# gaetanfacchinetti/DensityFlows.jl

Measured on AMD Instinct MI355X. Metric: forward+logdetJ Msamples/s, d=5 8-layer RealNVP, 1/2/4/8 MI355X, higher is better.
Workload: dtype f32

## Files before the change

densityflows.jl_amd/csrc/df_plan.cpp:

```cpp
#include "df_plan.h"

#include <algorithm>
#include <cmath>
#include <cstring>
#include <cstdlib>
#include <set>
#include <sstream>

namespace df {
namespace {

struct Fail {
    int code;
    std::string msg;
};

[[noreturn]] void fail(int code, const std::string& m) { throw Fail{code, m}; }

int round_up(int v, int m) { return (v + m - 1) / m * m; }

int pow2_tiles(int t) {
    int p = 1;
    while (p < t) p *= 2;
    return p;
// ... 47 lines not shown
private:
    Plan& P;
    int cap_;
    int cur_ = -1;
    int used_ = 0;
};

void check_net(const df_dense_desc* net, int nd, int in_dim, int out_dim, const char* which) {
    if (nd < 1) fail(DF_ERR_INVALID, std::string(which) + ": a conditioner needs at least one Dense");
    if (!net) fail(DF_ERR_INVALID, std::string(which) + ": null Dense array");
    int prev = in_dim;
    for (int k = 0; k < nd; ++k) {
        const df_dense_desc& D = net[k];
        if (D.in_dim != prev) {
            std::ostringstream os;
            os << which << ": Dense " << k + 1 << " expects " << D.in_dim << " inputs but receives " << prev;
            fail(DF_ERR_SHAPE, os.str());
        }
        if (D.out_dim < 1 || !D.W) fail(DF_ERR_INVALID, std::string(which) + ": empty Dense");
        if (D.act < DF_ACT_IDENTITY || D.act > DF_ACT_SWISH)
            fail(DF_ERR_INVALID, std::string(which) + ": unknown activation");
        if (k + 1 < nd && D.out_dim > kMaxHidden) fail(DF_ERR_UNSUPPORTED, "hidden width > 256");
        prev = D.out_dim;
    }
    if (prev != out_dim) {
        std::ostringstream os;
        os << which << ": output dimension " << prev << " does not match the " << out_dim
           << " transformed dimensions";
        fail(DF_ERR_SHAPE, os.str());
    }
}

void build_split(const df_chain_desc* desc, Plan& P, const std::vector<char>& fold) {
    P.split = 0;
    if (!P.fast || (P.ht != 2 && P.ht != 4)) return;
    const int ht = P.ht, H = 16 * ht;
    auto net_bytes = [&](int n_out) {
        return kSplitFirstBytes(ht) + kSplitHiddenBytes(ht) + 4 * H + round_up((n_out * H + 4) * 4, 16);
    };
    int total = 0, biggest = 0;
    for (const ULayer& U : P.ulayers) {
        if (U.kind == DF_LAYER_NORM) continue;
        const int b = net_bytes(U.t.n_out) + (U.kind == DF_LAYER_RNVP ? net_bytes(U.s.n_out) : 0);
        total += b;
        biggest = std::max(biggest, std::max(net_bytes(U.t.n_out), U.kind == DF_LAYER_RNVP ? net_bytes(U.s.n_out) : 0));
    }
    const int cap = total <= kSingleStageCap ? kSingleStageCap : std::max(kStageCap, round_up(biggest, kStageAlign));
    std::vector<uint8_t>& blob = P.sblob;
    int cur = -1, used = 0;
    auto close = [&]() {
        if (cur < 0) return;
        used = round_up(used, kStageAlign);
        blob.resize((size_t)P.sstages[cur].src_off + used, 0);
        P.sstages[cur].bytes = used;
        P.sstage_max = std::max(P.sstage_max, used);
    };
    auto alloc = [&](int bytes) {
        if (cur < 0 || used + bytes > cap) {
            close();
            cur = (int)P.sstages.size();
            DevStage s{};
            s.src_off = (int64_t)blob.size();
            P.sstages.push_back(s);
            used = 0;
        }
        const int off = used;
        used += bytes;
        blob.resize((size_t)P.sstages[cur].src_off + used, 0);
        return std::make_pair(cur, off);
    };
    P.sulayers = P.ulayers;
    for (int li = 0; li < desc->n_layers; ++li) {
        const df_layer_desc& L = desc->layers[li];
        if (L.kind == DF_LAYER_NORM) continue;
        const DevLayer& DL = P.layers[li];
        auto pack = [&](const df_dense_desc* net, int d0, UNet* u) {
            const DevDense &D0 = P.denses[d0], &D1 = P.denses[d0 + 1], &DO = P.denses[d0 + 2];
            auto [st, off] = alloc(net_bytes(u->n_out));
            u->stage = st;
            u->off_w0 = off;
            u->off_h = off + kSplitFirstBytes(ht);
            u->off_out = u->off_h + kSplitHiddenBytes(ht) + 4 * H;
            u->off_b0 = -1;
            u->hstride = 0;
            const int64_t base = P.sstages[st].src_off;
            auto put16 = [&](int64_t at, int32_t src, int plane, float v) {
                const uint16_t h = bf16_split_plane(v, plane);
                std::memcpy(&blob[base + at], &h, 2);
                if (src >= 0) {
                    P.spack_dst.push_back((int32_t)(base + at));
                    P.spack_src.push_back(src * 4 + plane);
                }
            };
            auto put32 = [&](int64_t at, int32_t src, float v) {
                std::memcpy(&blob[base + at], &v, 4);
                if (src >= 0) {
                    P.spack_dst.push_back((int32_t)(base + at));
                    P.spack_src.push_back(src * 4 + 3);
                }
            };
            const df_dense_desc& W0 = net[0];
            static const int kPlaneOfSlot[6] = {0, 0, 1, 0, 1, 2};
            for (int m = 0; m < ht; ++m)
                for (int lane = 0; lane < 64; ++lane) {
                    const int g = lane >> 4, row = 16 * m + (lane & 15);
                    float v = 0.f;
                    int32_t src = -1;
                    if (row < W0.out_dim) {
                        if (fold[li] && g == 3) {
                            v = W0.b[row];
                            src = D0.b_off + row;
                        } else if (g < W0.in_dim) {
                            v = W0.W[(size_t)row + (size_t)W0.out_dim * g];
                            src = D0.w_off + row + W0.out_dim * g;
                        }
                    }
                    for (int e = 0; e < 6; ++e)
                        put16(u->off_w0 + ((int64_t)m * 64 + lane) * 16 + 2 * e, src, kPlaneOfSlot[e], v);
                }
            const df_dense_desc& W1 = net[1];
            for (int c = 0; c < ht / 2; ++c)
                for (int m = 0; m < ht; ++m)
                    for (int p = 0; p < 3; ++p)
                        for (int lane = 0; lane < 64; ++lane)
                            for (int e = 0; e < 8; ++e) {
                                const int g = lane >> 4, row = 16 * m + (lane & 15);
                                const int k = 32 * c + 16 * (e >> 2) + 4 * g + (e & 3);
                                const bool ok = row < W1.out_dim && k < W1.in_dim;
                                put16(u->off_h + ((((int64_t)c * ht + m) * 3 + p) * 64 + lane) * 16 + 2 * e,
                                      ok ? D1.w_off + row + W1.out_dim * k : -1, p,
                                      ok ? W1.W[(size_t)row + (size_t)W1.out_dim * k] : 0.f);
                            }
            const int64_t hb = u->off_h + kSplitHiddenBytes(ht);
            for (int row = 0; row < H; ++row) {
                const bool ok = W1.b && row < W1.out_dim;
                put32(hb + 4 * row, ok ? D1.b_off + row : -1, ok ? W1.b[row] : 0.f);
            }
            const df_dense_desc& W2 = net[2];
            for (int o = 0; o < W2.out_dim; ++o)
                for (int k = 0; k < H; ++k) {
                    const bool ok = k < W2.in_dim;
                    put32(u->off_out + 4 * ((int64_t)o * H + k), ok ? DO.w_off + o + W2.out_dim * k : -1,
                          ok ? W2.W[(size_t)o + (size_t)W2.out_dim * k] : 0.f);
                }
            for (int o = 0; o < 4; ++o) {
                const bool ok = W2.b && o < W2.out_dim;
                put32(u->off_out + 4 * ((int64_t)W2.out_dim * H + o), ok ? DO.b_off + o : -1, ok ? W2.b[o] : 0.f);
            }
            P.split_flops_per_sample += 2.0 * (W0.in_dim * W0.out_dim + W1.in_dim * W1.out_dim);
        };
        ULayer& U = P.sulayers[li];
        if (L.kind == DF_LAYER_RNVP) pack(L.s_net, DL.s_dense0, &U.s);
        pack(L.t_net, DL.t_dense0, &U.t);
    }
    close();
    auto sched = [&](bool fwd) {
        std::vector<int32_t> out;
        auto push = [&](int s) {
            if (out.empty() || out.back() != s) out.push_back(s);
        };
        for (int it = 0; it < P.n_layers; ++it) {
            const ULayer& U = P.sulayers[fwd ? it : P.n_layers - 1 - it];
            if (U.kind == DF_LAYER_NORM) continue;
            if (fwd) {
                if (U.kind == DF_LAYER_RNVP) push(U.s.stage);
                push(U.t.stage);
            } else {
                push(U.t.stage);
                if (U.kind == DF_LAYER_RNVP) push(U.s.stage);
            }
        }
        return out;
    };
    P.ssched_fwd = sched(true);
    P.ssched_bwd = sched(false);
    int target = kLdsPerBlockTarget;
    if (const char* e = std::getenv("DF_SPLIT_LDS_KB")) target = std::max(32, std::atoi(e)) * 1024;
    const int nbuf = P.sstages.size() > 1 ? 2 : 1;
    const int fixed = nbuf * P.sstage_max + table_lds_bytes(P);
    const int per_tile = kWavesPerBlock * 16 * P.stride * 4;
    int t = 0;
    while (t < kMaxTilesPerWave && fixed + (t + 1) * per_tile <= target) ++t;
    t -= t % P.tile_group;
    if (t < P.tile_group) {
        P.sulayers.clear();
        P.sstages.clear();
        P.sblob.clear();
        P.spack_dst.clear();
        P.spack_src.clear();
        P.split_flops_per_sample = 0.0;
        return;
    }
    P.stiles = t;
    P.sblob.resize(round_up((int)P.sblob.size(), 16) + 16, 0);
    P.split = 1;
}

void build_wide(const df_chain_desc* desc, Plan& P) {
    if (const char* f = std::getenv("DF_NO_WIDE"))
        if (f[0] == '1') return;
    if (P.uniform || P.ht != 16) return;
    for (int li = 0; li < desc->n_layers; ++li) {
        const df_layer_desc& L = desc->layers[li];
        if (L.kind == DF_LAYER_NORM) continue;
        auto ok = [&](const df_dense_desc* net, int nd) {
            return nd == 3 && net[0].in_dim <= kMaxState && net[0].out_dim == 256 && net[1].out_dim == 256 &&
                   net[2].out_dim <= 32 && net[0].act == DF_ACT_RELU && net[1].act == DF_ACT_RELU &&
                   net[2].act == DF_ACT_IDENTITY;
        };
        if (L.kind == DF_LAYER_RNVP && !ok(L.s_net, L.n_dense_s)) return;
        if (!ok(L.t_net, L.n_dense_t)) return;
    }
    int li_dense = 0;
    std::vector<WLayer> wl;
    for (int li = 0; li < desc->n_layers; ++li) {
        const df_layer_desc& L = desc->layers[li];
        const DevLayer& DL = P.layers[li];
        WLayer W{};
        W.kind = DL.kind;
        W.elem_start = DL.elem_start;
        W.elem_end = DL.elem_end;
        W.n_af = DL.n_af;
        W.feat_tab = DL.feat_tab;
        W.af_tab = DL.af_tab;
        W.norm_off = DL.norm_off;
        W.alpha = DL.alpha;
        W.beta = DL.beta;
        W.ldj_const = DL.ldj_const;
        if (L.kind != DF_LAYER_NORM) {
            auto pack = [&](const df_dense_desc* net, int d0, WNet& N) {
                const int ks = (net[0].in_dim + 3) / 4;
                const int nkq0 = (ks + 3) / 4;
                N.stage0 = (int)P.wstages.size();
                N.nst0 = (nkq0 + 1) / 2;
                N.ks = ks;
                N.n_out = net[2].out_dim;
                N.mto = (N.n_out + 15) / 16;
                N.act0 = net[0].act;
                N.act1 = net[1].act;
                N.act_out = net[2].act;
                auto new_stage = [&](int bytes) -> float* {
                    DevStage st{};
                    st.src_off = (int64_t)P.wblob.size();
                    st.bytes = bytes;
                    P.wstages.push_back(st);
                    P.wblob.resize(P.wblob.size() + bytes, 0);
                    return reinterpret_cast<float*>(P.wblob.data() + st.src_off);
                };
                auto put = [&](float* base, int64_t q, int dense, int row, int k) {
                    const df_dense_desc& D = net[dense];
                    if (row >= D.out_dim || k >= D.in_dim) return;
                    base[q] = D.W[(size_t)row + (size_t)D.out_dim * k];
                    const int64_t f0 = (reinterpret_cast<uint8_t*>(base) - P.wblob.data()) / 4;
                    P.wpack_dst.push_back((int32_t)(f0 + q));
                    P.wpack_src.push_back(P.denses[d0 + dense].w_off + row + D.out_dim * k);
                };
                for (int st = 0; st < N.nst0; ++st) {
                    float* b = new_stage(kWideStageBytes);
                    for (int kk = 0; kk < 2; ++kk)
                        for (int m = 0; m < 16; ++m)
                            for (int lane = 0; lane < 64; ++lane)
                                for (int r = 0; r < 4; ++r) {
                                    const int s = 4 * (2 * st + kk) + r;
                                    if (s >= ks) continue;
                                    put(b, ((int64_t)(kk * 16 + m) * 64 + lane) * 4 + r, 0, 16 * m + (lane & 15),
                                        4 * s + (lane >> 4));
                                }
                }
                for (int st = 0; st < 8; ++st) {
                    float* b = new_stage(kWideStageBytes);
                    for (int kk = 0; kk < 2; ++kk)
                        for (int m = 0; m < 16; ++m)
                            for (int lane = 0; lane < 64; ++lane)
                                for (int r = 0; r < 4; ++r)
                                    put(b, ((int64_t)(kk * 16 + m) * 64 + lane) * 4 + r, 1, 16 * m + (lane & 15),
                                        16 * (2 * st + kk) + 4 * (lane >> 4) + r);
                }
                {
                    float* b = new_stage(16 * N.mto * 1024);
                    for (int kq = 0; kq < 16; ++kq)
                        for (int m = 0; m < N.mto; ++m)
                            for (int lane = 0; lane < 64; ++lane)
                                for (int r = 0; r < 4; ++r)
                                    put(b, ((int64_t)(kq * N.mto + m) * 64 + lane) * 4 + r, 2, 16 * m + (lane & 15),
                                        16 * kq + 4 * (lane >> 4) + r);
                }
                auto bias = [&](int dense, int rows) -> int32_t {
                    const df_dense_desc& D = net[dense];
                    const int32_t off = (int32_t)P.wbias.size();
                    P.wbias.resize(P.wbias.size() + rows, 0.f);
                    if (!D.b) return off;
                    for (int r = 0; r < D.out_dim; ++r) {
                        P.wbias[off + r] = D.b[r];
                        P.wbias_dst.push_back(off + r);
                        P.wbias_src.push_back(P.denses[d0 + dense].b_off + r);
                    }
                    return off;
                };
                N.b0 = bias(0, 256);
                N.b1 = bias(1, 256);
                N.bo = bias(2, 16 * N.mto);
            };
            if (L.kind == DF_LAYER_RNVP) pack(L.s_net, DL.s_dense0, W.s);
            pack(L.t_net, DL.t_dense0, W.t);
        }
        wl.push_back(W);
// ... 653 lines not shown
```

densityflows.jl_amd/csrc/df_plan.h:

```cpp
#pragma once

#include <cstdint>
#include <string>
#include <vector>

#include "densityflows_hip.h"

namespace df {

constexpr int kWave = 64;
#ifndef DF_BLOCK_WAVES
#define DF_BLOCK_WAVES 8
#endif
#ifndef DF_LDS_TARGET_KB
#define DF_LDS_TARGET_KB 80
#endif
constexpr int kBlockThreads = 64 * DF_BLOCK_WAVES;
constexpr int kWavesPerBlock = kBlockThreads / kWave;
constexpr int kMaxState = 64;
constexpr int kMaxHidden = 256;
constexpr int kMaxAf = 32;
constexpr int kMaxLayers = 4096;
constexpr int kStageCap = 24 * 1024;
constexpr int kSingleStageCap = 64 * 1024;
constexpr int kBigStageCap = 64 * 1024;
constexpr int kStageAlign = 1024;
constexpr int kMaxTableInts = 4096;
constexpr int kMaxTilesPerWave = 8;
#ifndef DF_UNI_TT
#define DF_UNI_TT 1
#endif
constexpr int kUniformTileGroup = DF_UNI_TT;
#ifndef DF_FAST_TT
#define DF_FAST_TT 2
#endif
constexpr int kFastTileGroup = DF_FAST_TT;
constexpr int kLdsPerBlockTarget = DF_LDS_TARGET_KB * 1024;

enum : int32_t { IN_STATE = 0, IN_HIDDEN = 1 };

struct DevChunk {
    int32_t stage, lds_off, kq_begin, kq_end;
};

struct DevDense {
    int32_t in_kind;
    int32_t ks;
    int32_t kt_in;
    int32_t mt;
    int32_t out_valu;
    int32_t n_out;
    int32_t act;
    int32_t has_bias;
    int32_t bias_stage, bias_lds;
    int32_t chunk0, n_chunks;
    int32_t w3_stage, w3_lds;
    int32_t compact;
    int32_t in_dim;
    int32_t w_off, b_off;
};

struct DevLayer {
    int32_t kind;
    int32_t elem_start;
    int32_t elem_end;
    int32_t n_af;
    int32_t feat_tab;
    int32_t af_tab;
    int32_t s_dense0, s_ndense;
    int32_t t_dense0, t_ndense;
    int32_t norm_off;
    int32_t out_valu;
    float alpha, beta, ldj_const, pad;
};

struct UNet {
    int32_t stage;
    int32_t ks;
    int32_t nh;
    int32_t n_out;
    int32_t off_w0, off_b0;
    int32_t off_h, hstride;
    int32_t off_out;
    int32_t act0, acth, act_out;
    int32_t fold0;
};

struct ULayer {
    int32_t kind, elem_start, elem_end, n_af;
    int32_t feat_tab, af_tab, norm_off, pad0;
    float alpha, beta, ldj_const, pad1;
    UNet s, t;
};

constexpr int kWideStageBytes = 32 * 1024;
#ifndef DF_WIDE_NB
#define DF_WIDE_NB 2
#endif
constexpr int kWideBufs = DF_WIDE_NB;
constexpr int kWideWaves = 4;
constexpr int kWideT = 2;
#ifndef DF_WSPLIT_HALF
#define DF_WSPLIT_HALF 0
#endif
constexpr int kWideSplitHalves = DF_WSPLIT_HALF ? 2 : 1;
constexpr int kWideSplitStageBytes = 48 * 1024 / kWideSplitHalves;
constexpr int kWideSplitBufs = DF_WSPLIT_HALF ? 4 : 2;

struct WNet {
    int32_t stage0;
    int32_t nst0;
    int32_t nso;
    int32_t ks;
    int32_t n_out, mto;
    int32_t act0, act1, act_out;
    int32_t b0, b1, bo;
};

struct WLayer {
    int32_t kind, elem_start, elem_end, n_af;
    int32_t feat_tab, af_tab, norm_off, pad0;
    float alpha, beta, ldj_const, pad1;
    WNet s, t;
};

struct DevStage {
    int64_t src_off;
    int32_t bytes;
    int32_t pad;
};

#if defined(__HIPCC__)
#define DF_HD __host__ __device__
#else
#define DF_HD
#endif
DF_HD inline uint16_t bf16_rne_bits(float f) {
    const uint32_t u = __builtin_bit_cast(uint32_t, f);
    if ((u & 0x7fffffffu) > 0x7f800000u) return (uint16_t)((u >> 16) | 0x40u);
    return (uint16_t)((u + 0x7fffu + ((u >> 16) & 1u)) >> 16);
}
DF_HD inline float bf16_bits_to_f32(uint16_t h) { return __builtin_bit_cast(float, (uint32_t)h << 16); }
DF_HD inline uint16_t bf16_split_plane(float w, int plane) {
    const uint16_t h0 = bf16_rne_bits(w);
    if (plane == 0) return h0;
    const float r = w - bf16_bits_to_f32(h0);
    const uint16_t h1 = bf16_rne_bits(r);
    if (plane == 1) return h1;
    return bf16_rne_bits(r - bf16_bits_to_f32(h1));
}
constexpr int kSplitFirstBytes(int ht) { return ht * 1024; }
constexpr int kSplitHiddenBytes(int ht) { return (ht / 2) * ht * 3 * 1024; }

struct Plan {
    int d = 0, n = 0, n_layers = 0;
    int stride = 0;
    int ht = 0;
    int tiles = 0;
    int outv = 0;
    int uniform = 0;
    int relu_only = 0;
    int tile_group = 1;
    int fast = 0;
    std::vector<ULayer> ulayers;
    int samples_per_block = 0;
    int stage_max = 0;
    std::vector<int32_t> sched_fwd;
    std::vector<int32_t> sched_bwd;
    std::vector<DevLayer> layers;
    std::vector<DevDense> denses;
    std::vector<DevChunk> chunks;
    std::vector<DevStage> stages;
    std::vector<uint8_t> blob;
    std::vector<int32_t> tables;
    std::vector<float> params;
    int64_t n_params = 0;
    std::vector<float> trainables;
    std::vector<int32_t> pack_dst, pack_src;
    int wide = 0;
    std::vector<WLayer> wlayers;
    std::vector<DevStage> wstages;
    std::vector<uint8_t> wblob;
    std::vector<float> wbias;
    std::vector<int32_t> wsched_fwd, wsched_bwd;
    std::vector<int32_t> wpack_dst, wpack_src;
    std::vector<int32_t> wbias_dst, wbias_src;
    int split = 0;
    int stiles = 0;
    int sstage_max = 0;
    std::vector<ULayer> sulayers;
    std::vector<DevStage> sstages;
    std::vector<uint8_t> sblob;
    std::vector<int32_t> ssched_fwd, ssched_bwd;
    std::vector<int32_t> spack_dst, spack_src;
    int wsplit = 0;
    std::vector<WLayer> wslayers;
    std::vector<DevStage> wsstages;
    std::vector<uint8_t> wsblob;
    std::vector<int32_t> wssched_fwd, wssched_bwd;
    std::vector<int32_t> wspack_dst, wspack_src;
    std::vector<int32_t> wstables;
    double flops_per_sample = 0.0;
    double split_flops_per_sample = 0.0;
};

int build_plan(const df_chain_desc* desc, Plan* out, std::string* err, int exact = -1);

size_t plan_lds_bytes(const Plan& p);
inline bool params_in_lds(const Plan& p) { return p.uniform && p.params.size() <= (size_t)kBlockThreads; }
inline int table_lds_ints(const Plan& p) { return (int)(p.tables.size() + (params_in_lds(p) ? p.params.size() : 0)); }
inline int table_lds_bytes(const Plan& p) { return (table_lds_ints(p) * 4 + 15) / 16 * 16; }

}
```

densityflows.jl_amd/csrc/df_uniform_impl.h:

```cpp
#pragma once

#include <type_traits>

#include "df_chain_impl.h"

namespace df {
namespace uni {


using impl::lds4;
using impl::mfma4;
using impl::Stager;

__device__ __forceinline__ float relu_fast(float x) {
    return __int_as_float(__builtin_elementwise_max(__float_as_int(x), 0));
}

__device__ __forceinline__ float xgroup_sum(float p) {
    auto a = __builtin_amdgcn_permlane16_swap(__float_as_uint(p), __float_as_uint(p), false, false);
    const float q = __uint_as_float(a[0]) + __uint_as_float(a[1]);
    auto b = __builtin_amdgcn_permlane32_swap(__float_as_uint(q), __float_as_uint(q), false, false);
    return __uint_as_float(b[0]) + __uint_as_float(b[1]);
}

// ... 455 lines not shown
            const bf16x8 w2 = *reinterpret_cast<const bf16x8*>(f + 2048);
#pragma unroll
            for (int t = 0; t < TT; ++t) {
                f32x4 a = out[t][m];
                a = mfma_bf(w2, x[t][0], a);
                a = mfma_bf(w1, x[t][1], a);
                a = mfma_bf(w0, x[t][2], a);
                a = mfma_bf(w1, x[t][0], a);
                a = mfma_bf(w0, x[t][1], a);
                out[t][m] = mfma_bf(w0, x[t][0], a);
            }
            if (FENCE) asm volatile("" ::: "memory");
        }
    }
}

#ifndef DF_SPLIT_PREFETCH
#define DF_SPLIT_PREFETCH 1
#endif

__device__ __forceinline__ void sched_fence() { __builtin_amdgcn_sched_barrier(0); }

__device__ __forceinline__ void lds_wait0() { __builtin_amdgcn_s_waitcnt(0xc07f); }

struct SplitStep {
    bf16x8 w0, w1, w2;
    f32x4 b;
};

template <int HT, bool BIAS>
__device__ __forceinline__ void split_step_request(const uint8_t* wl, const uint8_t* bl, int s, SplitStep& f) {
    if (s >= (HT / 2) * HT) return;
    const uint8_t* p = wl + s * 3072;
    f.w0 = *reinterpret_cast<const bf16x8*>(p);
    f.w1 = *reinterpret_cast<const bf16x8*>(p + 1024);
    f.w2 = *reinterpret_cast<const bf16x8*>(p + 2048);
    if (BIAS && s < HT) f.b = lds4(bl + (s << 6));
}

template <int HT, int TT, bool BIAS = true>
__device__ __forceinline__ void dense_hidden_split_pf(const uint8_t* wb, int lane, const f32x4 (&in)[TT][HT],
                                                      f32x4 (&out)[TT][HT], const SplitStep& f0) {
    const int g = lane >> 4;
    const uint8_t* bl = wb + (HT / 2) * HT * 3072 + (g << 4);
    const uint8_t* wl = wb + lane * 16;
    const short4v eye = neg_eye();
    SplitStep f[2];
    f[0] = f0;
    bf16x8 x[TT][3];
#pragma unroll
    for (int s = 0; s < (HT / 2) * HT; ++s) {
        const int c = s / HT, m = s % HT;
        if (m == 0) {
#pragma unroll
            for (int t = 0; t < TT; ++t) split8_mrem(eye, in[t][2 * c], in[t][2 * c + 1], x[t][0], x[t][1], x[t][2]);
        }
        constexpr int NS = (HT / 2) * HT;
        const bool late = (m == HT - 1) && (s + 1 < NS);
        sched_fence();
        lds_wait0();
        if (!late) split_step_request<HT, BIAS>(wl, bl, s + 1, f[(s + 1) & 1]);
        sched_fence();
        const SplitStep& w = f[s & 1];
#pragma unroll
        for (int t = 0; t < TT; ++t) {
            f32x4 a = c == 0 ? (BIAS ? w.b : f32x4{0.f, 0.f, 0.f, 0.f}) : out[t][m];
            a = mfma_bf(w.w2, x[t][0], a);
            a = mfma_bf(w.w1, x[t][1], a);
            a = mfma_bf(w.w0, x[t][2], a);
            a = mfma_bf(w.w1, x[t][0], a);
            a = mfma_bf(w.w0, x[t][1], a);
            out[t][m] = mfma_bf(w.w0, x[t][0], a);
        }
        if (late) {
#pragma unroll
            for (int t = 0; t < TT; ++t) asm volatile("" : "+v"(out[t][m]));
            sched_fence();
            split_step_request<HT, BIAS>(wl, bl, s + 1, f[(s + 1) & 1]);
        }
    }
}

template <int HT, int TT>
__device__ __forceinline__ void dense_first_split_pf(const bf16x8 (&w)[HT], const float (&xin)[TT][4],
                                                     f32x4 (&acc)[TT][HT]) {
    bf16x8 b[TT];
    const __bf16 z = (__bf16)0.f;
#pragma unroll
    for (int t = 0; t < TT; t += 2) {
        bf16x2 h, m, l;
        split2(xin[t][0], t + 1 < TT ? xin[t + 1][0] : 0.f, h, m, l);
        b[t] = bf16x8{h[0], m[0], h[0], l[0], m[0], h[0], z, z};
        if (t + 1 < TT) b[t + 1] = bf16x8{h[1], m[1], h[1], l[1], m[1], h[1], z, z};
    }
#pragma unroll
    for (int m = 0; m < HT; ++m)
#pragma unroll
        for (int t = 0; t < TT; ++t) acc[t][m] = mfma_bf(w[m], b[t], f32x4{0.f, 0.f, 0.f, 0.f});
}

template <int HT, int NO>
__device__ __forceinline__ void out_row_request(const uint8_t* w3g, int oo, f32x4 (&w)[HT]) {
    if (oo >= NO) return;
#pragma unroll
    for (int kq = 0; kq < HT; ++kq) w[kq] = lds4(w3g + ((oo * 16 * HT + 16 * kq) << 2));
}

template <int HT, int TT, int NO>
__device__ __forceinline__ void out_valu_t_pf(const uint8_t* w3g, const f32x4 (&w0)[HT], float bo,
                                              const f32x4 (&h)[TT][HT], const float* state, const int (&ro)[TT],
                                              const int& aslot, float (&v)[TT], float (&y)[TT]) {
    static_assert(NO >= 1 && NO <= 4, "FAST tails: 1..4 outputs");
    float p[TT][4];
#pragma unroll
    for (int t = 0; t < TT; ++t)
#pragma unroll
        for (int oo = 0; oo < 4; ++oo) p[t][oo] = 0.f;
    f32x4 w[2][HT];
#pragma unroll
    for (int kq = 0; kq < HT; ++kq) w[0][kq] = w0[kq];
#pragma unroll
    for (int oo = 0; oo < NO; ++oo) {
        sched_fence();
        lds_wait0();
        if (oo == 0) {
#pragma unroll
            for (int t = 0; t < TT; ++t) v[t] = state[ro[t] + aslot];
        }
        out_row_request<HT, NO>(w3g, oo + 1, w[(oo + 1) & 1]);
        sched_fence();
#pragma unroll
        for (int kq = 0; kq < HT; ++kq)
#pragma unroll
            for (int r = 0; r < 4; ++r)
#pragma unroll
                for (int t = 0; t < TT; ++t) p[t][oo] = __builtin_fmaf(w[oo & 1][kq][r], h[t][kq][r], p[t][oo]);
#pragma unroll
        for (int t = 0; t < TT; ++t) asm volatile("" : "+v"(p[t][oo]));
    }
#pragma unroll
    for (int t = 0; t < TT; ++t) {
        auto a = __builtin_amdgcn_permlane16_swap(__float_as_uint(p[t][0]), __float_as_uint(p[t][1]), false, false);
        const float A = __uint_as_float(a[0]) + __uint_as_float(a[1]);
        float Bv = 0.f;
        if constexpr (NO > 2) {
            auto b = __builtin_amdgcn_permlane16_swap(__float_as_uint(p[t][2]), __float_as_uint(p[t][3]), false, false);
            Bv = __uint_as_float(b[0]) + __uint_as_float(b[1]);
        }
        auto c = __builtin_amdgcn_permlane32_swap(__float_as_uint(A), __float_as_uint(Bv), false, false);
        y[t] = (__uint_as_float(c[0]) + __uint_as_float(c[1])) + bo;
    }
}

template <int HT, int TT, bool OUTV, bool RELU, int PH, bool FAST = false, int NO = 0, bool SPLIT = false>
__device__ __forceinline__ void net_tiles(const uint8_t* buf, const UNet& N, const ULayer& L, const int32_t* tab,
                                          float* state, const int (&ro)[TT], float (&sum)[TT]) {
    const int lane = threadIdx.x & 63, g = lane >> 4;
    constexpr bool SPH = (PH == impl::PH_S_FWD || PH == impl::PH_S_BWD);
#if DF_SPLIT_PREFETCH && !defined(DF_EXP_NOTAIL) && !defined(DF_DIAG_NOSPLIT)
    if constexpr (SPLIT && FAST && HT >= 2 && OUTV && NO > 0) {
        int tx = threadIdx.x;
        asm volatile("" : "+v"(tx));
        const int lane = tx & 63, g = lane >> 4;
        const int off_out = N.off_out, af_tab = L.af_tab;
        asm volatile("" ::"s"(off_out), "s"(af_tab));
        const int slot = tab[L.feat_tab + g];
        bf16x8 w0[HT];
#pragma unroll
        for (int m = 0; m < HT; ++m) w0[m] = *reinterpret_cast<const bf16x8*>(buf + N.off_w0 + lane * 16 + m * 1024);
        sched_fence();
        lds_wait0();
        float xin[TT][4];
#pragma unroll
        for (int t = 0; t < TT; ++t) xin[t][0] = state[ro[t] + slot];
        const uint8_t* wh = buf + N.off_h;
        SplitStep f0;
        split_step_request<HT, true>(wh + lane * 16, wh + (HT / 2) * HT * 3072 + (g << 4), 0, f0);
        sched_fence();
        f32x4 A[TT][HT], B[TT][HT];
        dense_first_split_pf<HT, TT>(w0, xin, A);
        bias_act<HT, TT, true>(buf, DF_ACT_RELU, A, false);
        dense_hidden_split_pf<HT, TT>(wh, lane, A, B, f0);
        const uint8_t* w3g = buf + off_out + (g << 4);
        sched_fence();
        f32x4 wo[HT];
        out_row_request<HT, NO>(w3g, 0, wo);
        const float bo = reinterpret_cast<const float*>(buf + off_out)[NO * 16 * HT + (g < NO ? g : 0)];
        const int aslot = tab[af_tab + (g < NO ? g : 0)];
        sched_fence();
        bias_act<HT, TT, true>(buf, DF_ACT_RELU, B, false);
        float v[TT], y[TT];
        out_valu_t_pf<HT, TT, NO>(w3g, wo, bo, B, state, ro, aslot, v, y);
#pragma unroll
        for (int t = 0; t < TT; ++t) {
            if (g < NO) state[ro[t] + aslot] = couple1<PH>(v[t], y[t]);
            sum[t] = SPH ? group_row_sum<NO>(y[t]) : 0.f;
        }
        return;
    }
#endif
    if constexpr (SPLIT && FAST && HT >= 2) {
        float xin[TT][4];
        const int slot = tab[L.feat_tab + g];
#pragma unroll
        for (int t = 0; t < TT; ++t) xin[t][0] = state[ro[t] + slot];
        f32x4 A[TT][HT], B[TT][HT];
        dense_first_split<HT, TT>(buf, N, xin, A);
        bias_act<HT, TT, true>(buf, DF_ACT_RELU, A, false);
        dense_hidden_split<HT, TT>(buf + N.off_h, A, B);
        bias_act<HT, TT, true>(buf, DF_ACT_RELU, B, false);
        tail<HT, TT, OUTV, RELU, PH, NO>(buf, N, L, tab, state, ro, sum, B);
        return;
    }
    float xin[TT][4];
    const int32_t* feat = tab + L.feat_tab;
    constexpr int KS = FAST ? 1 : 0;
    const int ks = FAST ? 1 : N.ks;
#pragma unroll
    for (int r = 0; r < 4; ++r) {
        const int slot = (r < ks) ? feat[4 * r + g] : 0;
#pragma unroll
        for (int t = 0; t < TT; ++t) xin[t][r] = (r < ks) ? state[ro[t] + slot] : 0.f;
    }

    f32x4 A[TT][HT], B[TT][HT];
    dense_first<HT, TT, KS>(buf, N, xin, A);
    bias_act<HT, TT, RELU>(buf + N.off_b0, N.act0, A, FAST ? false : !N.fold0);
    if (FAST || N.nh == 1) {
        dense_hidden<HT, TT>(buf + N.off_h, A, B);
        bias_act<HT, TT, RELU>(buf + N.off_h + HT * HT * 1024, N.acth, B);
        tail<HT, TT, OUTV, RELU, PH, NO>(buf, N, L, tab, state, ro, sum, B);
        return;
    }
    bool in_a = true;
    for (int k = 0; k < N.nh; k += 2) {
        dense_hidden<HT, TT>(buf + N.off_h + k * N.hstride, A, B);
        bias_act<HT, TT, RELU>(buf + N.off_h + k * N.hstride + HT * HT * 1024, N.acth, B);
        in_a = false;
        if (k + 1 < N.nh) {
            dense_hidden<HT, TT>(buf + N.off_h + (k + 1) * N.hstride, B, A);
            bias_act<HT, TT, RELU>(buf + N.off_h + (k + 1) * N.hstride + HT * HT * 1024, N.acth, A);
            in_a = true;
        }
    }
    if (in_a) tail<HT, TT, OUTV, RELU, PH, NO>(buf, N, L, tab, state, ro, sum, A);
    else tail<HT, TT, OUTV, RELU, PH, NO>(buf, N, L, tab, state, ro, sum, B);
}

template <int HT, int TT, bool RELU, bool FWDP, int NO>
__device__ __forceinline__ void net_pair_tiles(const uint8_t* buf, const ULayer& L, const int32_t* tab, float* state,
                                               const int (&ro)[TT], float (&ssum)[TT]) {
    const int lane = threadIdx.x & 63, g = lane >> 4;
    float xin[TT][4];
    const int slot_in = tab[L.feat_tab + g];
#pragma unroll
    for (int t = 0; t < TT; ++t) xin[t][0] = state[ro[t] + slot_in];
    f32x4 As[TT][HT], At[TT][HT], Bs[TT][HT], Bt[TT][HT];
    dense_first<HT, TT, 1>(buf, L.s, xin, As);
    dense_first<HT, TT, 1>(buf, L.t, xin, At);
    bias_act<HT, TT, RELU>(buf + L.s.off_b0, L.s.act0, As, false);
    bias_act<HT, TT, RELU>(buf + L.t.off_b0, L.t.act0, At, false);
    dense_hidden<HT, TT>(buf + L.s.off_h, As, Bs);
    dense_hidden<HT, TT>(buf + L.t.off_h, At, Bt);
    bias_act<HT, TT, RELU>(buf + L.s.off_h + HT * HT * 1024, L.s.acth, Bs);
    bias_act<HT, TT, RELU>(buf + L.t.off_h + HT * HT * 1024, L.t.acth, Bt);
    float ys[TT], yt[TT];
    out_valu_t<HT, TT, NO>(buf, L.s, Bs, ys);
    out_valu_t<HT, TT, NO>(buf, L.t, Bt, yt);
    const int slot = tab[L.af_tab + (g < NO ? g : 0)];
#pragma unroll
    for (int t = 0; t < TT; ++t) {
        if (g < NO) {
            float v = state[ro[t] + slot];
            if (FWDP) {
                v = v * expf(ys[t]);
                v = v + yt[t];
            } else {
                v = v - yt[t];
                v = v * expf(-ys[t]);
            }
            state[ro[t] + slot] = v;
        }
        ssum[t] = group_row_sum<NO>(ys[t]);
    }
}

}

#ifndef DF_UNI_WAVES
#define DF_UNI_WAVES 4
#endif
#ifndef DF_FAST_WAVES
#define DF_FAST_WAVES 4
#endif

template <int HT, int MODE, bool OUTV, bool RELU, bool FAST = false, bool SPLIT = false>
__global__ void __launch_bounds__(kBlockThreads, FAST ? DF_FAST_WAVES : DF_UNI_WAVES)
uniform_kernel(ChainArgs a) {
    using namespace uni;
    constexpr bool FWD = (MODE == MODE_FWD || MODE == MODE_FWD_INPLACE);
    constexpr bool WANT_LDJ = (MODE != MODE_FWD_INPLACE);

    extern __shared__ __attribute__((aligned(16))) uint8_t smem[];
    const int stage_area = a.stage_bytes * a.n_stage_bufs;
    int32_t* tab = reinterpret_cast<int32_t*>(smem + stage_area);
    float* state = reinterpret_cast<float*>(smem + stage_area + a.tab_bytes);

    ClockStamp clk;
    clk.begin(a);
#ifdef DF_PHASE_STAMPS
    uint64_t ph[16] = {};
#define DF_PH(i) do { if (blockIdx.x == 0 && threadIdx.x == 0) ph[i] = __builtin_amdgcn_s_memtime(); } while (0)
#else
#define DF_PH(i) do {} while (0)
#endif
    DF_PH(0);
    const int tid = threadIdx.x;
    const int lane = tid & 63, wave = tid >> 6;
    const int g = lane >> 4, j = lane & 15;
    const int d = a.d, n = a.n, stride = a.stride, nd = n + d;
    const int nt = a.tiles;
    const int S = kWavesPerBlock * 16 * nt;
    const int cA = nd + 1, cE = nd + 2;
    const int64_t s0 = (int64_t)blockIdx.x * S;
    const int nvalid = (int)((a.batch - s0) < S ? (a.batch - s0) : S);

    Stager sg;
    sg.base = smem;
    sg.bytes = a.stage_bytes;
    sg.sched = FWD ? a.sched_fwd : a.sched_bwd;
    sg.n = FWD ? a.n_sched_fwd : a.n_sched_bwd;
    constexpr bool kLaneLocalDma = SPLIT && DF_SPLIT_PREFETCH;
    impl::stager_start<kLaneLocalDma>(sg, a);

    float* tabf = reinterpret_cast<float*>(tab);
    constexpr int kRowMax = 8;
    const bool fast_copy = d <= kRowMax && n <= kRowMax && a.n_par <= kBlockThreads && a.tab_ints <= 4 * kBlockThreads;
    auto row_init = [&](int smp) {
        for (int c = nd; c < stride; ++c) state[smp * stride + c] = (c == nd + 3) ? 1.f : 0.f;
    };
    auto theta_in = [&](float v, float lo, float hi) {
        const float diff = hi - lo;
        return (diff == 0.f) ? 0.f : (v - lo) / diff;
    };
    if (fast_copy) {
        const int n_tab = a.tab_ints, n_par = a.n_par;
        int tv[4];
#pragma unroll
        for (int u = 0; u < 4; ++u) {
            const int i = tid + u * kBlockThreads;
            tv[u] = i < n_tab ? a.tables[i] : 0;
        }
        const float pv = tid < n_par ? a.params[tid] : 0.f;
        const bool norm_th = a.tmin != nullptr;
        const float blo = (norm_th && lane < n) ? a.tmin[lane] : 0.f;
        const float bhi = (norm_th && lane < n) ? a.tmax[lane] : 0.f;
        const int smp = tid;
        const bool valid = smp < nvalid;
        float zr[kRowMax], tr[kRowMax];
#pragma unroll
        for (int c = 0; c < kRowMax; ++c)
            if (c < d) zr[c] = valid ? a.zin[(s0 + smp) * d + c] : 0.f;
#pragma unroll
        for (int c = 0; c < kRowMax; ++c)
            if (c < n) tr[c] = valid ? a.theta[(s0 + smp) * n + c] : 0.f;
#pragma unroll
        for (int u = 0; u < 4; ++u) {
            const int i = tid + u * kBlockThreads;
            if (i < n_tab) tab[i] = tv[u];
        }
        if (tid < n_par) tabf[n_tab + tid] = pv;
#pragma unroll
        for (int c = 0; c < kRowMax; ++c)
            if (c < n) {
                const float lo = __shfl(blo, c), hi = __shfl(bhi, c);
                if (smp < S) state[smp * stride + c] = (norm_th && valid) ? theta_in(tr[c], lo, hi) : tr[c];
            }
        if (smp < S) {
#pragma unroll
            for (int c = 0; c < kRowMax; ++c)
                if (c < d) state[smp * stride + n + c] = zr[c];
            row_init(smp);
        }
        for (int i = tid + kBlockThreads * d; i < S * d; i += kBlockThreads) {
            const int r = i / d, c = i - r * d;
            state[r * stride + n + c] = r < nvalid ? a.zin[(s0 + r) * d + c] : 0.f;
        }
        for (int i = tid + kBlockThreads * n; i < S * n; i += kBlockThreads) {
            const int r = i / n, c = i - r * n;
            float v = 0.f;
            if (r < nvalid) {
                v = a.theta[(s0 + r) * n + c];
                if (norm_th) v = theta_in(v, a.tmin[c], a.tmax[c]);
            }
            state[r * stride + c] = v;
        }
        for (int r = tid + kBlockThreads; r < S; r += kBlockThreads) row_init(r);
    } else {
        for (int i = tid; i < a.tab_ints; i += kBlockThreads) tab[i] = a.tables[i];
        for (int i = tid; i < S * d; i += kBlockThreads) {
            const int smp = i / d, c = i - smp * d;
            float v = 0.f;
            if (smp < nvalid) v = a.zin[(s0 + smp) * d + c];
            state[smp * stride + n + c] = v;
        }
        for (int i = tid; i < S * n; i += kBlockThreads) {
            const int smp = i / n, c = i - smp * n;
            float v = 0.f;
            if (smp < nvalid) {
                v = a.theta[(s0 + smp) * n + c];
                if (a.tmin) v = theta_in(v, a.tmin[c], a.tmax[c]);
            }
            state[smp * stride + c] = v;
        }
        for (int i = tid; i < S; i += kBlockThreads) row_init(i);
    }
    DF_PH(1);
    DF_PH(2);
    DF_PH(3);
    __syncthreads();
    DF_PH(4);

    const int row0 = ((wave * nt) * 16 + j) * stride;
#ifdef DF_NO_PAIR
    constexpr bool no_pair = true;
#else
    constexpr bool no_pair = false;
#endif
    const int tstep = 16 * stride;
    bool have_acc = false;

    auto ldj_update = [&](int ro, float l, bool first_in_elem, bool last_in_elem) {
        if (!WANT_LDJ || g != 0) return;
        const float e = first_in_elem ? l : state[ro + cE] + l;
        state[ro + cE] = e;
        if (last_in_elem) state[ro + cA] = have_acc ? state[ro + cA] + e : e;
    };

    for (int it = 0; it < a.n_layers; ++it) {
        const int li = FWD ? it : a.n_layers - 1 - it;
        using CULayer = const __attribute__((address_space(4))) ULayer;
#ifdef DF_PHASE_STAMPS
        const ULayer L = *(const ULayer*)(&((CULayer*)(uintptr_t)a.ulayers)[li]);
        asm volatile("s_waitcnt lgkmcnt(0)" ::: "memory");
        if (it == 1) DF_PH(13);
#else
        const ULayer& L = *(const ULayer*)(&((CULayer*)(uintptr_t)a.ulayers)[li]);
#endif
        const int kind = L.kind;
        const bool first_in_elem = FWD ? L.elem_start : L.elem_end;
        const bool last_in_elem = FWD ? L.elem_end : L.elem_start;
        int gl = g, jl = j, wavel = wave, row0l = row0;
        if constexpr (kLaneLocalDma) {
            if (kind == DF_LAYER_NORM || (!FWD && a.snap)) {
                int tx = tid;
                asm volatile("" : "+v"(tx));
                gl = (tx & 63) >> 4, jl = tx & 15, wavel = tx >> 6;
                row0l = ((wavel * nt) * 16 + jl) * stride;
            }
        }
        if (kind == DF_LAYER_NORM) {
            const float al = L.alpha, be = L.beta, delta = be - al;
            auto norm = [&](const auto* xmn) {
                const auto* xmx = xmn + d;
                for (int tt = 0; tt < nt; ++tt) {
                    const int ro = row0l + tt * tstep;
                    for (int i = gl; i < d; i += 4) {
                        const float lo = xmn[i], hi = xmx[i], xd = hi - lo;
                        float v = state[ro + n + i];
                        if (FWD) v = ((xd * v - al * hi) + be * lo) / delta;
                        else v = (be * (v - lo) + al * (hi - v)) / xd;
                        state[ro + n + i] = v;
                    }
                    ldj_update(ro, FWD ? L.ldj_const : -L.ldj_const, first_in_elem, last_in_elem);
                }
            };
            if (fast_copy) norm(tabf + a.tab_ints + L.norm_off);
            else norm(a.params + L.norm_off);
        } else {
            const bool rnvp = (kind == DF_LAYER_RNVP);
            constexpr int kTT = FAST ? kFastTileGroup : kUniformTileGroup;
            auto tiles_loop = [&](const UNet& N, auto ph_tag, auto no_tag, bool sphase, float sign) {
                constexpr int PH = decltype(ph_tag)::value;
                constexpr int NO = decltype(no_tag)::value;
                const uint8_t* buf = sg.buf();
                for (int tt = 0; tt < nt; tt += kTT) {
                    int ro[kTT];
                    float ssum[kTT];
                    int r0 = row0;
                    if constexpr (SPLIT) asm volatile("" : "+v"(r0));
#pragma unroll
                    for (int t = 0; t < kTT; ++t) ro[t] = r0 + (tt + t) * tstep;
                    net_tiles<HT, kTT, OUTV, RELU, PH, FAST, NO, SPLIT>(buf, N, L, tab, state, ro, ssum);
#pragma unroll
                    for (int t = 0; t < kTT; ++t) {
                        if (sphase) ldj_update(ro[t], sign * ssum[t], first_in_elem, last_in_elem);
                        else if (!rnvp) ldj_update(ro[t], 0.f, first_in_elem, last_in_elem);
                    }
                }
            };
            auto run_net = [&](const UNet& N, auto ph_tag, bool sphase, float sign) {
                impl::ensure_stage<kLaneLocalDma>(N.stage, sg, a);
                if constexpr (FAST && OUTV) {
                    switch (N.n_out) {
                        case 1: tiles_loop(N, ph_tag, std::integral_constant<int, 1>{}, sphase, sign); break;
                        case 2: tiles_loop(N, ph_tag, std::integral_constant<int, 2>{}, sphase, sign); break;
                        case 3: tiles_loop(N, ph_tag, std::integral_constant<int, 3>{}, sphase, sign); break;
                        default: tiles_loop(N, ph_tag, std::integral_constant<int, 4>{}, sphase, sign); break;
                    }
                } else {
                    tiles_loop(N, ph_tag, std::integral_constant<int, 0>{}, sphase, sign);
                }
            };
            using PSF = std::integral_constant<int, impl::PH_S_FWD>;
            using PTF = std::integral_constant<int, impl::PH_T_FWD>;
            using PTB = std::integral_constant<int, impl::PH_T_BWD>;
            using PSB = std::integral_constant<int, impl::PH_S_BWD>;
            bool paired = false;
            if constexpr (FAST && OUTV && !SPLIT && HT <= 2) {
                if (rnvp && L.s.stage == L.t.stage && L.s.n_out == L.t.n_out && !no_pair) {
                    impl::ensure_stage(L.s.stage, sg, a);
                    auto pair_loop = [&](auto no_tag) {
                        constexpr int NO = decltype(no_tag)::value;
                        const uint8_t* buf = sg.buf();
                        for (int tt = 0; tt < nt; tt += kTT) {
                            int ro[kTT];
                            float ssum[kTT];
#pragma unroll
                            for (int t = 0; t < kTT; ++t) ro[t] = row0 + (tt + t) * tstep;
                            net_pair_tiles<HT, kTT, RELU, FWD, NO>(buf, L, tab, state, ro, ssum);
#pragma unroll
                            for (int t = 0; t < kTT; ++t)
                                ldj_update(ro[t], FWD ? ssum[t] : -ssum[t], first_in_elem, last_in_elem);
                        }
                    };
                    switch (L.s.n_out) {
                        case 1: pair_loop(std::integral_constant<int, 1>{}); break;
                        case 2: pair_loop(std::integral_constant<int, 2>{}); break;
                        case 3: pair_loop(std::integral_constant<int, 3>{}); break;
                        default: pair_loop(std::integral_constant<int, 4>{}); break;
                    }
                    paired = true;
                }
            }
            if (paired) {
            } else if (FWD) {
#ifdef DF_PHASE_STAMPS
                if (it == 1) DF_PH(11);
#endif
                if (rnvp) run_net(L.s, PSF{}, true, 1.f);
#ifdef DF_PHASE_STAMPS
                if (it == 1) DF_PH(12);
#endif
                run_net(L.t, PTF{}, false, 1.f);
            } else {
                run_net(L.t, PTB{}, false, 1.f);
                if (rnvp) run_net(L.s, PSB{}, true, -1.f);
            }
        }
        have_acc = have_acc || last_in_elem;
#ifdef DF_PHASE_STAMPS
        if (it == 0) DF_PH(5);
        if (it == 1) DF_PH(6);
        if (it == 2) DF_PH(7);
        if (it == 3) DF_PH(8);
#endif
        if (!FWD && a.snap) {
            float* dst = a.snap + (int64_t)li * a.batch * d;
            for (int tt = 0; tt < nt; ++tt) {
                const int smp = (wavel * nt + tt) * 16 + jl;
                if (smp < nvalid)
                    for (int i = gl; i < d; i += 4) dst[(s0 + smp) * d + i] = state[row0l + tt * tstep + n + i];
            }
        }
    }

    asm volatile("s_waitcnt vmcnt(0)" ::: "memory");
    if (MODE == MODE_LOGPDF) {
        double part = 0.0;
        if (g == 0) {
            for (int tt = 0; tt < nt; ++tt) {
                const int ro = row0 + tt * tstep;
                const int smp = (wave * nt + tt) * 16 + j;
                float q = 0.f;
                for (int i = 0; i < d; ++i) {
                    const float zz = state[ro + n + i];
                    q = q + zz * zz;
                }
                const float lp = (a.c0 - q / 2.f) + state[ro + cA];
                if (smp < nvalid) {
                    if (a.lp_out) a.lp_out[s0 + smp] = lp;
                    part += (double)lp;
                }
            }
        }
        if (a.partial) {
#pragma unroll
            for (int off = 32; off >= 1; off >>= 1) part += __shfl_xor(part, off);
            __syncthreads();
            double* red = reinterpret_cast<double*>(smem);
            if (lane == 0) red[wave] = part;
            __syncthreads();
            if (tid == 0) {
                double s = 0.0;
                for (int w = 0; w < kWavesPerBlock; ++w) s += red[w];
                a.partial[blockIdx.x] = s;
            }
        }
        if (!a.xout) {
            clk.end(a);
            return;
        }
    }
    __syncthreads();
    for (int i = tid; i < S * d; i += kBlockThreads) {
        const int smp = i / d, c = i - smp * d;
        if (smp < nvalid) a.xout[(s0 + smp) * d + c] = state[smp * stride + n + c];
    }
    if (WANT_LDJ && MODE != MODE_LOGPDF && a.ldj_out) {
        for (int i = tid; i < nvalid; i += kBlockThreads) a.ldj_out[s0 + i] = state[i * stride + cA];
    }
    DF_PH(9);
#ifdef DF_PHASE_STAMPS
    asm volatile("s_waitcnt vmcnt(0)" ::: "memory");
    DF_PH(10);
    if (blockIdx.x == 0 && threadIdx.x == 0) {
#pragma unroll
        for (int i = 1; i < 14; ++i) a.xout[i] = (float)(ph[i] - ph[0]);
    }
#endif
#undef DF_PH
    clk.end(a);
}

template <int HT, bool RELU, bool FAST = false, bool SPLIT = false>
void* uniform_kernel_ptr_r(int mode, bool outv) {
#define DF_U(M) (outv ? reinterpret_cast<void*>(&uniform_kernel<HT, M, true, RELU, FAST, SPLIT>) \
                      : reinterpret_cast<void*>(&uniform_kernel<HT, M, false, RELU, FAST, SPLIT>))
    switch (mode) {
        case MODE_FWD: return DF_U(MODE_FWD);
        case MODE_FWD_INPLACE: return DF_U(MODE_FWD_INPLACE);
        case MODE_BWD: return DF_U(MODE_BWD);
        default: return DF_U(MODE_LOGPDF);
    }
#undef DF_U
}

template <int HT>
void* uniform_kernel_ptr(int mode, int variant) {
    const bool outv = variant & 1;
    if constexpr (HT >= 2) {
        if ((variant & 8) && (variant & 4) && outv) return uniform_kernel_ptr_r<HT, true, true, true>(mode, true);
    }
    if (variant & 8) return nullptr;
    if (variant & 4) return uniform_kernel_ptr_r<HT, true, true>(mode, outv);
    return (variant & 2) ? uniform_kernel_ptr_r<HT, true>(mode, outv) : uniform_kernel_ptr_r<HT, false>(mode, outv);
}

template <int HT>
hipError_t launch_uniform_ht(int mode, int variant, const ChainArgs& a, unsigned grid, size_t lds, hipStream_t st) {
    void* args[] = {const_cast<ChainArgs*>(&a)};
    return hipLaunchKernel(uniform_kernel_ptr<HT>(mode, variant), dim3(grid), dim3(kBlockThreads), args, lds, st);
}

// ... 21 lines not shown
```

Baseline: 1617.

## Pack split-path slot tables into scalar words and add wave priority hints

For the SPLIT fast path, the planner now packs the four feature and affine slot indices into 8-bit fields of two 32-bit words stored in the former ULayer padding. It also checks that the net layout matches compile-time offsets. The kernel keeps these words and the weight offset in scalar registers and decodes each slot with a shift, instead of loading per-lane table entries from LDS or global memory. The hidden-layer weight request is issued before the first LDS wait, and s_setprio raises wave priority during the matrix phase. The main risks are the added 8-bit slot limit, extra plan validation failures, and the scheduling effect of the priority changes.

Result: faster. 1660, median of 6 (+2.7%).

```diff
diff --git a/densityflows.jl_amd/csrc/df_plan.cpp b/densityflows.jl_amd/csrc/df_plan.cpp
--- a/densityflows.jl_amd/csrc/df_plan.cpp
+++ b/densityflows.jl_amd/csrc/df_plan.cpp
@@ -223,6 +223,18 @@
         ULayer& U = P.sulayers[li];
         if (L.kind == DF_LAYER_RNVP) pack(L.s_net, DL.s_dense0, &U.s);
         pack(L.t_net, DL.t_dense0, &U.t);
+        for (int g = 0; g < 4; ++g) {
+            const int32_t f = P.tables[U.feat_tab + g], a = P.tables[U.af_tab + (g < U.n_af ? g : 0)];
+            if (f < 0 || f >= (1 << kSplitSlotBits) || a < 0 || a >= (1 << kSplitSlotBits))
+                fail(DF_ERR_UNSUPPORTED, "SPLIT plan: a state slot does not fit the 8 bits of a slot word");
+        }
+        U.feat_word = split_feat_word(P.tables.data(), U);
+        U.af_word = split_af_word(P.tables.data(), U);
+        for (const UNet* u : {&U.s, &U.t}) {
+            if (u == &U.s && L.kind != DF_LAYER_RNVP) continue;
+            if (u->off_h != u->off_w0 + kSplitOffH(ht) || u->off_out != u->off_w0 + kSplitOffOut(ht))
+                fail(DF_ERR_INVALID, "internal: SPLIT net layout differs from kSplitOffH / kSplitOffOut");
+        }
     }
     close();
     auto sched = [&](bool fwd) {
diff --git a/densityflows.jl_amd/csrc/df_plan.h b/densityflows.jl_amd/csrc/df_plan.h
--- a/densityflows.jl_amd/csrc/df_plan.h
+++ b/densityflows.jl_amd/csrc/df_plan.h
@@ -88,10 +88,26 @@
 
 struct ULayer {
     int32_t kind, elem_start, elem_end, n_af;
-    int32_t feat_tab, af_tab, norm_off, pad0;
-    float alpha, beta, ldj_const, pad1;
+    int32_t feat_tab, af_tab, norm_off;
+    int32_t feat_word;
+    float alpha, beta, ldj_const;
+    int32_t af_word;
     UNet s, t;
 };
+static_assert(sizeof(ULayer) == 12 * 4 + 2 * sizeof(UNet), "ULayer: the slot words take the former pads");
+
+constexpr int kSplitSlotBits = 8;
+inline int32_t split_feat_word(const int32_t* tables, const ULayer& U) {
+    uint32_t w = 0;
+    for (int g = 0; g < 4; ++g) w |= (uint32_t)(tables[U.feat_tab + g] & 0xff) << (kSplitSlotBits * g);
+    return (int32_t)w;
+}
+inline int32_t split_af_word(const int32_t* tables, const ULayer& U) {
+    uint32_t w = 0;
+    for (int g = 0; g < 4; ++g)
+        w |= (uint32_t)(tables[U.af_tab + (g < U.n_af ? g : 0)] & 0xff) << (kSplitSlotBits * g);
+    return (int32_t)w;
+}
 
 constexpr int kWideStageBytes = 32 * 1024;
 #ifndef DF_WIDE_NB
@@ -151,6 +167,8 @@
 }
 constexpr int kSplitFirstBytes(int ht) { return ht * 1024; }
 constexpr int kSplitHiddenBytes(int ht) { return (ht / 2) * ht * 3 * 1024; }
+constexpr int kSplitOffH(int ht) { return kSplitFirstBytes(ht); }
+constexpr int kSplitOffOut(int ht) { return kSplitFirstBytes(ht) + kSplitHiddenBytes(ht) + 4 * 16 * ht; }
 
 struct Plan {
     int d = 0, n = 0, n_layers = 0;
diff --git a/densityflows.jl_amd/csrc/df_uniform_impl.h b/densityflows.jl_amd/csrc/df_uniform_impl.h
--- a/densityflows.jl_amd/csrc/df_uniform_impl.h
+++ b/densityflows.jl_amd/csrc/df_uniform_impl.h
@@ -631,41 +631,61 @@
     }
 }
 
+struct SplitHead {
+    int off_w0, feat_word, af_word;
+};
+#if DF_SPLIT_PREFETCH && !defined(DF_EXP_NOTAIL) && !defined(DF_DIAG_NOSPLIT)
+#define DF_SPLIT_HEAD_REGS 1
+#else
+#define DF_SPLIT_HEAD_REGS 0
+#endif
+
+#ifndef DF_SPLIT_PRIO
+#define DF_SPLIT_PRIO 1
+#endif
+template <bool MATRIX_PHASE>
+__device__ __forceinline__ void split_prio() {
+    if constexpr (DF_SPLIT_PRIO == 1) __builtin_amdgcn_s_setprio(MATRIX_PHASE ? 2 : 0);
+    if constexpr (DF_SPLIT_PRIO == 2) __builtin_amdgcn_s_setprio(MATRIX_PHASE ? 0 : 2);
+}
+
 template <int HT, int TT, bool OUTV, bool RELU, int PH, bool FAST = false, int NO = 0, bool SPLIT = false>
 __device__ __forceinline__ void net_tiles(const uint8_t* buf, const UNet& N, const ULayer& L, const int32_t* tab,
-                                          float* state, const int (&ro)[TT], float (&sum)[TT]) {
+                                          float* state, const int (&ro)[TT], float (&sum)[TT], const SplitHead& hd) {
     const int lane = threadIdx.x & 63, g = lane >> 4;
     constexpr bool SPH = (PH == impl::PH_S_FWD || PH == impl::PH_S_BWD);
-#if DF_SPLIT_PREFETCH && !defined(DF_EXP_NOTAIL) && !defined(DF_DIAG_NOSPLIT)
+#if DF_SPLIT_HEAD_REGS
     if constexpr (SPLIT && FAST && HT >= 2 && OUTV && NO > 0) {
         int tx = threadIdx.x;
         asm volatile("" : "+v"(tx));
         const int lane = tx & 63, g = lane >> 4;
-        const int off_out = N.off_out, af_tab = L.af_tab;
-        asm volatile("" ::"s"(off_out), "s"(af_tab));
-        const int slot = tab[L.feat_tab + g];
+        const uint8_t* net = buf + hd.off_w0;
+        const int slot = ((uint32_t)hd.feat_word >> (kSplitSlotBits * g)) & ((1 << kSplitSlotBits) - 1);
         bf16x8 w0[HT];
 #pragma unroll
-        for (int m = 0; m < HT; ++m) w0[m] = *reinterpret_cast<const bf16x8*>(buf + N.off_w0 + lane * 16 + m * 1024);
+        for (int m = 0; m < HT; ++m) w0[m] = *reinterpret_cast<const bf16x8*>(net + lane * 16 + m * 1024);
+        float xin[TT][4];
+#pragma unroll
+        for (int t = 0; t < TT; ++t) xin[t][0] = state[ro[t] + slot];
+        const uint8_t* wh = net + kSplitOffH(HT);
+        SplitStep f0;
+        split_step_request<HT, true>(wh + lane * 16, wh + (HT / 2) * HT * 3072 + (g << 4), 0, f0);
         sched_fence();
         lds_wait0();
-        float xin[TT][4];
-#pragma unroll
-        for (int t = 0; t < TT; ++t) xin[t][0] = state[ro[t] + slot];
-        const uint8_t* wh = buf + N.off_h;
-        SplitStep f0;
-        split_step_request<HT, true>(wh + lane * 16, wh + (HT / 2) * HT * 3072 + (g << 4), 0, f0);
+        split_prio<true>();
         sched_fence();
         f32x4 A[TT][HT], B[TT][HT];
         dense_first_split_pf<HT, TT>(w0, xin, A);
         bias_act<HT, TT, true>(buf, DF_ACT_RELU, A, false);
         dense_hidden_split_pf<HT, TT>(wh, lane, A, B, f0);
-        const uint8_t* w3g = buf + off_out + (g << 4);
+        const uint8_t* w3 = net + kSplitOffOut(HT);
+        const uint8_t* w3g = w3 + (g << 4);
         sched_fence();
+        split_prio<false>();
         f32x4 wo[HT];
         out_row_request<HT, NO>(w3g, 0, wo);
-        const float bo = reinterpret_cast<const float*>(buf + off_out)[NO * 16 * HT + (g < NO ? g : 0)];
-        const int aslot = tab[af_tab + (g < NO ? g : 0)];
+        const float bo = reinterpret_cast<const float*>(w3)[NO * 16 * HT + (g < NO ? g : 0)];
+        const int aslot = ((uint32_t)hd.af_word >> (kSplitSlotBits * g)) & ((1 << kSplitSlotBits) - 1);
         sched_fence();
         bias_act<HT, TT, true>(buf, DF_ACT_RELU, B, false);
         float v[TT], y[TT];
@@ -810,6 +830,7 @@
     sg.sched = FWD ? a.sched_fwd : a.sched_bwd;
     sg.n = FWD ? a.n_sched_fwd : a.n_sched_bwd;
     constexpr bool kLaneLocalDma = SPLIT && DF_SPLIT_PREFETCH;
+    constexpr bool kSplitHead = SPLIT && FAST && OUTV && HT >= 2 && DF_SPLIT_HEAD_REGS;
     impl::stager_start<kLaneLocalDma>(sg, a);
 
     float* tabf = reinterpret_cast<float*>(tab);
@@ -959,7 +980,8 @@
         } else {
             const bool rnvp = (kind == DF_LAYER_RNVP);
             constexpr int kTT = FAST ? kFastTileGroup : kUniformTileGroup;
-            auto tiles_loop = [&](const UNet& N, auto ph_tag, auto no_tag, bool sphase, float sign) {
+            auto tiles_loop = [&](const UNet& N, const SplitHead& hd, auto ph_tag, auto no_tag, bool sphase,
+                                  float sign) {
                 constexpr int PH = decltype(ph_tag)::value;
                 constexpr int NO = decltype(no_tag)::value;
                 const uint8_t* buf = sg.buf();
@@ -970,7 +992,7 @@
                     if constexpr (SPLIT) asm volatile("" : "+v"(r0));
 #pragma unroll
                     for (int t = 0; t < kTT; ++t) ro[t] = r0 + (tt + t) * tstep;
-                    net_tiles<HT, kTT, OUTV, RELU, PH, FAST, NO, SPLIT>(buf, N, L, tab, state, ro, ssum);
+                    net_tiles<HT, kTT, OUTV, RELU, PH, FAST, NO, SPLIT>(buf, N, L, tab, state, ro, ssum, hd);
 #pragma unroll
                     for (int t = 0; t < kTT; ++t) {
                         if (sphase) ldj_update(ro[t], sign * ssum[t], first_in_elem, last_in_elem);
@@ -979,16 +1001,22 @@
                 }
             };
             auto run_net = [&](const UNet& N, auto ph_tag, bool sphase, float sign) {
-                impl::ensure_stage<kLaneLocalDma>(N.stage, sg, a);
+                SplitHead hd{0, 0, 0};
+                int stage = N.stage, n_out = N.n_out;
+                if constexpr (kSplitHead) {
+                    hd = SplitHead{N.off_w0, L.feat_word, L.af_word};
+                    asm volatile("" : "+s"(stage), "+s"(n_out), "+s"(hd.off_w0), "+s"(hd.feat_word), "+s"(hd.af_word));
+                }
+                impl::ensure_stage<kLaneLocalDma>(stage, sg, a);
                 if constexpr (FAST && OUTV) {
-                    switch (N.n_out) {
-                        case 1: tiles_loop(N, ph_tag, std::integral_constant<int, 1>{}, sphase, sign); break;
-                        case 2: tiles_loop(N, ph_tag, std::integral_constant<int, 2>{}, sphase, sign); break;
-                        case 3: tiles_loop(N, ph_tag, std::integral_constant<int, 3>{}, sphase, sign); break;
-                        default: tiles_loop(N, ph_tag, std::integral_constant<int, 4>{}, sphase, sign); break;
+                    switch (n_out) {
+                        case 1: tiles_loop(N, hd, ph_tag, std::integral_constant<int, 1>{}, sphase, sign); break;
+                        case 2: tiles_loop(N, hd, ph_tag, std::integral_constant<int, 2>{}, sphase, sign); break;
+                        case 3: tiles_loop(N, hd, ph_tag, std::integral_constant<int, 3>{}, sphase, sign); break;
+                        default: tiles_loop(N, hd, ph_tag, std::integral_constant<int, 4>{}, sphase, sign); break;
                     }
                 } else {
-                    tiles_loop(N, ph_tag, std::integral_constant<int, 0>{}, sphase, sign);
+                    tiles_loop(N, hd, ph_tag, std::integral_constant<int, 0>{}, sphase, sign);
                 }
             };
             using PSF = std::integral_constant<int, impl::PH_S_FWD>;
```
